# LingmaFuture/PRCV2025REID

Hardware: AMD Instinct MI355X
Metric: multimodal instances/sec (PxK, 5-modality) at 1/2/4/8 GPU; eval queries/sec (higher is better)
Workload: dtype bf16; 1 GPU; P=16,K=4 per GPU, vis/nir/sk/cp 224x224 + text (T<=77), CLIP ViT-B/16 + text tower random-init, MER-LoRA r=8, masks all-on, 400 ids, SDM+CE, fwd+bwd+grad sanitise/clip+AdamW (reference default trainable set); P=16, K=4, global_batch=64, lora_rank=8, accum_steps=1, parallelism=dp1

## Files before the change

include/reid_hip.h:

```cpp
#ifndef REID_HIP_H
#define REID_HIP_H

#include <stdint.h>

#ifdef __cplusplus
extern "C" {
#endif

typedef enum {
    REID_OK = 0,
    REID_ERR_ARG = -1,
    REID_ERR_LAUNCH = -2,
    REID_ERR_DEVICE = -3
} reid_status;

typedef enum { REID_BF16 = 0, REID_F32 = 1, REID_F16 = 2 } reid_dtype;

typedef enum {
    REID_ACT_NONE = 0,
    REID_ACT_GELU_ERF = 1,
    REID_ACT_QUICK_GELU = 2,
    REID_ACT_RELU = 3,
    REID_ACT_DGELU_ERF = 4,
    REID_ACT_DQUICK_GELU = 5,
// ... 69 lines not shown

int reid_attn_fwd(const void* qkv, int32_t ld, const uint8_t* key_mask, void* out, int32_t ldo, float* lse,
                  int32_t n_seq, int32_t S, int32_t heads, int32_t causal, int32_t q_tiles, void* stream);
int reid_attn_bwd(const void* qkv, int32_t ld, const uint8_t* key_mask, const void* out, const void* dout,
                  int32_t ldo, const float* lse, void* dqkv, int32_t lddqkv, float* delta_ws,
                  int32_t n_seq, int32_t S, int32_t heads, int32_t causal, int32_t q_tiles, void* stream);

int reid_cast_f32_bf16(const float* src, void* dst, int64_t n, void* stream);
int reid_cast_bf16_f32(const void* src, float* dst, int64_t n, void* stream);
int reid_pack_bf16_table(const float* src, void* dst_bf16, const int64_t* table, int32_t n_entries, void* stream);
int reid_lora_bwd_fused(const void* dY, int32_t lddy, const void* T, int32_t ldt, const void* BT, int32_t ldbt, void* U, int32_t ldu,
                        float* dB, int32_t lddb, const int32_t* img_mod, int32_t rows_per_img, int32_t mask_r, int32_t M, int32_t N,
                        int32_t Rp, float scale, float* u_partial, int32_t u_mode, void* stream);
int reid_lora_da_fused(const void* X, int32_t ldx, const void* U, int32_t ldu, float* dA, int32_t ldda, const int32_t* img_mod,
                       int32_t rows_per_img, int32_t mask_r, int32_t M, int32_t K, int32_t Rp, int32_t n_groups, void* stream);

int reid_merge_lora_table(const int64_t* table, int32_t n_entries, int32_t max_tiles, const float* arena, void* weff,
                          int32_t Rp, int32_t r, int32_t nmod, float scaling, void* stream);
int reid_gather_rows_f32(const float* src, int32_t lds, const int32_t* index, float* dst, int32_t ldd,
                         int32_t rows, int32_t cols, void* stream);
int reid_embed_tokens(const float* tok, const float* pos, const int64_t* ids, float* out, int32_t B, int32_t T, int32_t D,
                      int32_t vocab, void* stream);
int reid_scatter_add_rows_f32(const float* src, int32_t lds, const int32_t* index, float* out, int32_t ldo,
                              int32_t rows, int32_t cols, int32_t out_rows, void* stream);

int reid_bnneck_stats(const float* x, int32_t ldx, int32_t rows, int32_t D, float* sum, float* sqsum, void* stream);
int reid_bnneck_fwd(const float* x, int32_t ldx, const float* gamma, const float* beta, float* running_mean,
                    float* running_var, const float* sum, const float* sqsum, float count, int32_t training,
                    float* y, void* y_bf16, int32_t ldy, float* mean, float* invstd, float* rnorm,
                    int32_t rows, int32_t D, float eps, float momentum, float scale, void* stream);
// ... 224 lines not shown
```

prcv2025reid_amd/_lib.py:

```python
import ctypes as C
import os

import torch

_HERE = os.path.dirname(os.path.abspath(__file__))
LIB_PATHS = {'bf16': os.path.join(_HERE, 'csrc', 'libreid_hip.so'), 'f16': os.path.join(_HERE, 'csrc', 'libreid_hip_f16.so')}
if os.environ.get('REID_LIB_BF16'):
    LIB_PATHS['bf16'] = os.environ['REID_LIB_BF16']
LIB_PATH = LIB_PATHS['bf16']
T16_DTYPES = {'bf16': torch.bfloat16, 'f16': torch.float16}
_flavor = os.environ.get('REID_T16', 'bf16')


def set_flavor(name: str):
    global _flavor
    if name not in LIB_PATHS:
        raise ValueError(f'unknown 16-bit flavor {name!r}')
    _flavor = name


def flavor() -> str:
    return _flavor


# ... 45 lines not shown
    'reid_mer_gemm': (_I, [_GEMM, _P]),
    'reid_mer_gemm_plan': (_I, [_GEMM, _I, _I, _PLAN]),
    'reid_gemm_tn': (_I, [_P, _P, _P, _I, _I, _I, _I, _I, _I, _F, _F, _P]),
    'reid_layernorm_fwd': (_I, [_P, _I, _P, _P, _P, _P, _P, _I, _P, _P, _I, _I, _F, _P]),
    'reid_add_layernorm_fwd': (_I, [_P, _I, _P, _I, _I, _P, _I, _P, _I, _P, _P, _P, _I, _P, _P, _I, _I, _F, _P]),
    'reid_layernorm_bwd': (_I, [_P, _I, _I, _P, _I, _P, _P, _P, _P, _P, _P, _I, _P, _I, _P, _P, _I, _I, _P, _I, _P, _P]),
    'reid_patch_im2col': (_I, [_P, _P, _I, _I, _I, _I, _I, _P]),
    'reid_cls_rows': (_I, [_P, _P, _P, _I, _I, _I, _I, _P]),
    'reid_attn_fwd': (_I, [_P, _I, _P, _P, _I, _P, _I, _I, _I, _I, _I, _P]),
    'reid_attn_bwd': (_I, [_P, _I, _P, _P, _P, _I, _P, _P, _I, _P, _I, _I, _I, _I, _I, _P]),
    'reid_cast_f32_bf16': (_I, [_P, _P, _I64, _P]),
    'reid_cast_bf16_f32': (_I, [_P, _P, _I64, _P]),
    'reid_pack_bf16_table': (_I, [_P, _P, _P, _I, _P]),
    'reid_lora_bwd_fused': (_I, [_P, _I, _P, _I, _P, _I, _P, _I, _P, _I, _P, _I, _I, _I, _I, _I, _F, _P, _I, _P]),
    'reid_lora_da_fused': (_I, [_P, _I, _P, _I, _P, _I, _P, _I, _I, _I, _I, _I, _I, _P]),
    'reid_merge_lora_table': (_I, [_P, _I, _I, _P, _P, _I, _I, _I, _F, _P]),
    'reid_gather_rows_f32': (_I, [_P, _I, _P, _P, _I, _I, _I, _P]),
    'reid_embed_tokens': (_I, [_P, _P, _P, _P, _I, _I, _I, _I, _P]),
    'reid_scatter_add_rows_f32': (_I, [_P, _I, _P, _P, _I, _I, _I, _I, _P]),
    'reid_bnneck_stats': (_I, [_P, _I, _I, _I, _P, _P, _P]),
    'reid_bnneck_fwd': (_I, [_P, _I, _P, _P, _P, _P, _P, _P, _F, _I, _P, _P, _I, _P, _P, _P, _I, _I, _F, _F, _F, _P]),
    'reid_bnneck_bwd_p1': (_I, [_P, _I, _P, _I, _P, _P, _P, _P, _P, _P, _P, _P, _I, _I, _F, _P]),
    'reid_bnneck_bwd_p2': (_I, [_P, _P, _I, _P, _P, _P, _P, _P, _F, _I, _P, _I, _I, _I, _P]),
    'reid_ce_ls_fwd': (_I, [_P, _I, _P, _P, _I, _I, _F, _P, _P, _P]),
    'reid_ce_ls_bwd': (_I, [_P, _I, _P, _P, _I, _I, _F, _P, _P, _I, _P]),
    'reid_sdm_fwd': (_I, [_P, _I, _P, _I, _P, _P, _P, _P, _I, _I, _I, _I, _F, _P, _P, _P]),
    'reid_sdm_bwd': (_I, [_P, _I, _P, _I, _P, _P, _P, _P, _I, _I, _I, _I, _F, _P, _P, _P, _I, _P, _I, _P]),
    'reid_sdm_ws_floats': (_I64, [_I, _I, _I, _I]),
    'reid_triplet_hard_fwd': (_I, [_P, _I, _P, _P, _I, _I, _F, _P, _P, _P, _P, _P, _P, _P]),
    'reid_triplet_hard_bwd': (_I, [_P, _I, _I, _I, _F, _P, _P, _P, _P, _P, _P, _P, _I, _P]),
# ... 147 lines not shown
```

prcv2025reid_amd/csrc/lora.hip:

```cpp
#include "lds_tile.h"
#include <type_traits>

namespace {
using namespace ldstile;

constexpr int MT = 64;

__global__ __launch_bounds__(256) void merge_lora_kernel(const int64_t* __restrict__ table, const float* __restrict__ arena,
                                                         bf16_t* __restrict__ weff, int Rp, int r, int nmod, float s) {
    REID_T16_ENTER();
    const int64_t* e = table + (size_t)blockIdx.y * 8;
    const int N = (int)e[5], K = (int)e[6], G = (int)e[7];
    const int tiles_k = K / MT;
    if ((int)blockIdx.x >= (N / MT) * tiles_k) return;
    const float* __restrict__ W = (const float*)e[0];
    const float* __restrict__ A = arena + e[1];
    const float* __restrict__ B = arena + e[2];
    bf16_t* dst = weff + e[3];
    bf16_t* dstT = e[4] >= 0 ? weff + e[4] : nullptr;
    const int n0 = ((int)blockIdx.x / tiles_k) * MT, k0 = ((int)blockIdx.x % tiles_k) * MT;
    const int g = n0 / (N / G);
    const int R = nmod * r;
    __shared__ __attribute__((aligned(16))) float sW[MT][MT + 4];
    __shared__ __attribute__((aligned(16))) float sA[MT][MT + 4];
// ... 274 lines not shown
    return buf + 1 == NBUF ? 0 : buf + 1;
}

__global__ __launch_bounds__(256) void u_finish_kernel(const float* __restrict__ Up, bf16_t* __restrict__ U, int ldu, const int32_t* __restrict__ img_mod,
                                                       int rows_per_img, int mask_r, float scale, int M, int Rp) {
    REID_T16_ENTER();
    const int i = blockIdx.x * 256 + threadIdx.x;
    const int h = Rp >> 1;
    const int m = i / h, c = (i - m * h) * 2;
    if (m >= M) return;
    const int mu = img_mod[m / rows_per_img];
    const float a = Up[(size_t)m * Rp + c], b = Up[(size_t)m * Rp + c + 1];
    *(uint32_t*)(U + (size_t)m * ldu + c) = pack_bf16x2(c / mask_r == mu ? a * scale : 0.f, (c + 1) / mask_r == mu ? b * scale : 0.f);
}

template <int RP>
__device__ __forceinline__ void lora_bwd_image_run(const Params& p, char* smem, const int rbeg, const int rend, const int mu) {
    constexpr int BUF_BYTES = BwdGeo<RP>::BUF_BYTES;
    int tid = threadIdx.x;
    asm volatile("" : "+v"(tid));
    const int lane = tid & 63;
    const int w = __builtin_amdgcn_readfirstlane(tid >> 6);
    const int l16 = lane & 15, fq = lane >> 4;
    const int w0 = (mu * p.mask_r) & ~15;
    const int c_lo = mu * p.mask_r - w0, c_hi = c_lo + p.mask_r;
    const int steps = (rend - rbeg + R - 1) / R;
    const uint32_t smem_a = lds_addr(smem);
    auto issue = [&](int t, int buf) {
        const uint32_t base = smem_a + buf * BUF_BYTES;
        const int r0 = rbeg + t * R;
        dma_tile(p.dY, p.lddy, r0, rend, w, lane, base);
        if constexpr (RP == 32) {
            if (w < 2) {
                const int g = w * 64 + lane;
                const int row = g >> 2, c = g & 3;
                int gr = r0 + row; gr = gr < rend ? gr : rend - 1;
                dma16(p.T + (size_t)gr * p.ldt + c * 8, base + IMG_BYTES + w * 1024);
            }
        } else {
            if (w == 0) {
                const int row = lane >> 1, c = lane & 1;
                int gr = r0 + row; gr = gr < rend ? gr : rend - 1;
                dma16(p.T + (size_t)gr * p.ldt + w0 + c * 8, base + IMG_BYTES);
            }
        }
    };
    ring_prologue(steps, issue);
    bf16x8 bfr[24];
    if (w < 2) {
#pragma unroll
        for (int ks = 0; ks < 24; ++ks) bfr[ks] = *(const bf16x8*)(p.BT + (size_t)(w0 + l16) * p.ldbt + ks * 32 + 8 * fq);
#pragma unroll
        for (int ks = 0; ks < 24; ++ks) asm volatile("" ::"v"(bfr[ks]));
    }
    f32x4 acc[8];
#pragma unroll
    for (int i = 0; i < 8; ++i) acc[i] = f32x4{0.f, 0.f, 0.f, 0.f};
    typedef unsigned u32x4_t __attribute__((ext_vector_type(4)));
    u32x4_t pend_val = u32x4_t{0u, 0u, 0u, 0u};
    u32x4_t pend_val2 = u32x4_t{0u, 0u, 0u, 0u};
    void* pend_ptr = nullptr;
    int pend_n = 0;
    if constexpr (RP == 64) {
        if (w < 2 && p.u_mode == 0) {
            char* ub = smem + NBUF * BUF_BYTES + w * (16 * RP * 2);
            *(u32x4_t*)(ub + lane * 16) = u32x4_t{0u, 0u, 0u, 0u};
            *(u32x4_t*)(ub + 1024 + lane * 16) = u32x4_t{0u, 0u, 0u, 0u};
        }
    }
    auto flush_pending = [&]() {
        if (p.u_mode == 0) {
            if constexpr (RP == 32) {
                if (pend_n) asm volatile("global_store_dwordx4 %0, %1, off" ::"v"(pend_ptr), "v"(pend_val) : "memory");
            } else {
                if (pend_n & 1) asm volatile("global_store_dwordx4 %0, %1, off" ::"v"(pend_ptr), "v"(pend_val) : "memory");
                if (pend_n & 2) {
                    void* pp2 = (void*)((bf16_t*)pend_ptr + (size_t)8 * p.ldu);
                    asm volatile("global_store_dwordx4 %0, %1, off" ::"v"(pp2), "v"(pend_val2) : "memory");
                }
            }
        } else {
#pragma unroll
            for (int e = 0; e < 4; ++e) {
                if (e >= pend_n) continue;
                float* pp = (float*)pend_ptr + (size_t)e * RP;
                const unsigned vv = pend_val[e];
                if (p.u_mode == 2) asm volatile("global_store_dword %0, %1, off" ::"v"(pp), "v"(vv) : "memory");
                else asm volatile("global_atomic_add_f32 %0, %1, off" ::"v"(pp), "v"(vv) : "memory");
            }
        }
        pend_n = 0;
    };
    int buf = 0;
    for (int t = 0; t < steps; ++t) {
        ring_wait(t, steps, w < (RP == 32 ? 2 : 1));
        const char* xs = smem + buf * BUF_BYTES;
        const char* ts = xs + IMG_BYTES;
        const int r0 = rbeg + t * R;
        if (w < 2) {
            flush_pending();
            f32x4 u4[4];
#pragma unroll
            for (int a = 0; a < 4; ++a) u4[a] = f32x4{0.f, 0.f, 0.f, 0.f};
            const int row = 16 * w + l16;
            const char* xrow = xs + row * ROW_BYTES;
#pragma unroll
            for (int k0 = 0; k0 < 24; k0 += 4) {
                bf16x8 af[4];
#pragma unroll
                for (int a = 0; a < 4; ++a) af[a] = *(const bf16x8*)(xrow + (swz512(row, 4 * (k0 + a) + fq) << 4));
#pragma unroll
                for (int a = 0; a < 4; ++a) u4[a] = mfma16(af[a], bfr[k0 + a], u4[a]);
            }
            const f32x4 ua = (u4[0] + u4[1]) + (u4[2] + u4[3]);
// ... 28 lines not shown
        } else {
            bf16x8 tf = RP == 32 ? tr_frag(ts, RP * 2, 0, w0, lane) : tr_frag(ts, 32, 0, 0, lane);
            const int nvalid = rend - r0;
            if (nvalid < R) {
#pragma unroll
                for (int j = 0; j < 8; ++j) {
                    if (16 * (j >> 2) + 4 * fq + (j & 3) >= nvalid) tf[j] = 0;
                }
            }
            const int cbase = (w - 2) * 128;
#pragma unroll
            for (int i = 0; i < 8; ++i) acc[i] = mfma16(tr_frag_swz(xs, cbase + i * 16, lane), tf, acc[i]);
        }
        buf = ring_refill(t, steps, buf, issue);
    }
    if (w < 2) flush_pending();
    __syncthreads();
    int ftid = threadIdx.x;
    asm volatile("" : "+v"(ftid));
    float* fl = (float*)smem;
    if (w >= 2) {
        const int cbase = (w - 2) * 128, fl16 = ftid & 15, ffq = (ftid & 63) >> 4;
#pragma unroll
        for (int i = 0; i < 8; ++i)
#pragma unroll
            for (int e = 0; e < 4; ++e) fl[(cbase + i * 16 + 4 * ffq + e) * 16 + fl16] = acc[i][e];
    }
    __syncthreads();
    {
        const int rr = p.mask_r, total = N * rr;
        for (int idx = ftid; idx < total; idx += 512) {
            const int col = idx / rr, j = idx - col * rr;
            atomicAdd(p.dB + (size_t)col * p.lddb + mu * rr + j, fl[col * 16 + c_lo + j]);
        }
    }
}

template <int RP>
__global__ __launch_bounds__(512, 2) void lora_bwd_image_kernel(const Params p) {
    REID_T16_ENTER();
    static_assert(RP == 32 || RP == 64, "adapter columns");
    extern __shared__ __attribute__((aligned(16))) char smem[];
    for_each_run(p, [=](int rbeg, int rend, int mu, bool more) { lora_bwd_image_run<RP>(p, smem, rbeg, rend, mu); if (more) __syncthreads(); });
}

struct DaParams {
    const bf16_t* X; const bf16_t* U; float* dA;
    const int32_t* img_mod;
    int ldx, ldu, ldda, rows_per_img, mask_r, M, Rp, span, n_img;
};
template <int G>
__device__ __forceinline__ void lora_da_image_run(const DaParams& p, char* smem, const int rbeg, const int rend, const int mu, const bool more) {
    constexpr int UB = 4096;
    constexpr int BUF = IMG_BYTES + UB;
    const int tid = threadIdx.x, lane = tid & 63;
    const int w = __builtin_amdgcn_readfirstlane(tid >> 6);
    const int l16 = lane & 15, fq = lane >> 4;
    const int cblk = blockIdx.y;
    const int w0 = (mu * p.mask_r) & ~15;
    const int c_lo = mu * p.mask_r - w0, c_hi = c_lo + p.mask_r;
    const int steps = (rend - rbeg + R - 1) / R;
    const bf16_t* Xb = p.X + (size_t)cblk * N;
    const uint32_t smem_a = lds_addr(smem);
    auto issue = [&](int t, int buf) {
        const uint32_t base = smem_a + buf * BUF;
        const int r0 = rbeg + t * R;
        dma_tile(Xb, p.ldx, r0, rend, w, lane, base);
        if (w < G) {
            const int row = lane >> 1, c = lane & 1;
            int gr = r0 + row; gr = gr < rend ? gr : rend - 1;
            dma16(p.U + (size_t)gr * p.ldu + w * p.Rp + w0 + c * 8, base + IMG_BYTES + w * 1024);
        }
    };
    ring_prologue(steps, issue);
    f32x4 acc[G][6];
#pragma unroll
    for (int g = 0; g < G; ++g)
#pragma unroll
        for (int i = 0; i < 6; ++i) acc[g][i] = f32x4{0.f, 0.f, 0.f, 0.f};
    int buf = 0;
    for (int t = 0; t < steps; ++t) {
        ring_wait(t, steps, w < G);
        const char* xs = smem + buf * BUF;
        const char* us = xs + IMG_BYTES;
        const int nvalid = rend - (rbeg + t * R);
        bf16x8 uf[G];
#pragma unroll
        for (int g = 0; g < G; ++g) {
            uf[g] = tr_frag(us + g * 1024, 32, 0, 0, lane);
            if (nvalid < R) {
#pragma unroll
                for (int j = 0; j < 8; ++j)
                    if (16 * (j >> 2) + 4 * fq + (j & 3) >= nvalid) uf[g][j] = 0;
            }
        }
#pragma unroll
        for (int i = 0; i < 6; ++i) {
            const bf16x8 xf = tr_frag_swz(xs, w * 96 + i * 16, lane);
#pragma unroll
            for (int g = 0; g < G; ++g) acc[g][i] = mfma16(uf[g], xf, acc[g][i]);
        }
        buf = ring_refill(t, steps, buf, issue);
    }
    if (more) __syncthreads();
#pragma unroll
    for (int e = 0; e < 4; ++e) {
        const int c = 4 * fq + e;
        if (c < c_lo || c >= c_hi) continue;
#pragma unroll
        for (int g = 0; g < G; ++g)
#pragma unroll
            for (int i = 0; i < 6; ++i)
                atomicAdd(p.dA + (size_t)(g * p.Rp + w0 + c) * p.ldda + (size_t)cblk * N + w * 96 + i * 16 + l16, acc[g][i][e]);
    }
}

template <int G>
__global__ __launch_bounds__(512, 2) void lora_da_image_kernel(const DaParams p) {
    REID_T16_ENTER();
    extern __shared__ __attribute__((aligned(16))) char smem[];
    for_each_run(p, [=](int rbeg, int rend, int mu, bool more) { lora_da_image_run<G>(p, smem, rbeg, rend, mu, more); });
}
}

}

static int lora_span(int n_img) {
    const int k = reid_knob(KNOB_LORA_SPAN);
    if (k == 1 || k == 2 || k == 4 || k == 8) return k;
    return n_img >= reid_num_cus() ? 4 : 1;
}

static bool lora_image_shape(int rows_per_img, int mask_r) { return rows_per_img >= image::R && mask_r <= 16 && 16 % mask_r == 0; }

extern "C" int reid_lora_bwd_fused(const void* dY, int32_t lddy, const void* T, int32_t ldt, const void* BT, int32_t ldbt, void* U,
                                   int32_t ldu, float* dB, int32_t lddb, const int32_t* img_mod, int32_t rows_per_img, int32_t mask_r,
                                   int32_t M, int32_t N, int32_t Rp, float scale, float* u_partial, int32_t u_mode, void* stream) {
    REID_CHECK_ARG(u_mode >= 0 && u_mode <= 3 && (u_mode == 0 || u_partial), "reid_lora_bwd_fused: u_mode=%d needs u_partial", u_mode);
    REID_CHECK_ARG(dY && T && BT && U && dB && img_mod, "reid_lora_bwd_fused: null pointer");
    REID_CHECK_ARG(N == fused::N && (Rp == 32 || Rp == 64), "reid_lora_bwd_fused: N=%d Rp=%d (this kernel is built for N = 768, Rp = 32 or 64)", N, Rp);
    REID_CHECK_ARG(M > 0 && rows_per_img > 0 && mask_r > 0 && mask_r <= Rp, "reid_lora_bwd_fused: M=%d rows_per_img=%d mask_r=%d", M, rows_per_img, mask_r);
    REID_CHECK_ARG(lddy % 8 == 0 && ldt % 8 == 0 && ldbt % 8 == 0 && ldu % 2 == 0 && lddy >= N && ldt >= Rp && ldbt >= N && ldu >= Rp && lddb >= Rp,
                   "reid_lora_bwd_fused: leading dimensions");
    REID_CHECK_ARG(((uintptr_t)dY | (uintptr_t)T | (uintptr_t)BT) % 16 == 0 && (uintptr_t)U % 4 == 0, "reid_lora_bwd_fused: operand alignment");
    fused::Params p{(const bf16_t*)dY, (const bf16_t*)T, (const bf16_t*)BT, (bf16_t*)U, dB, img_mod, lddy, ldt, ldbt, ldu, lddb, rows_per_img,
                    mask_r, M, 0, scale, u_partial, u_mode, 1, 0};
    const bool use_image = reid_knob(KNOB_LORA_IMPL) != 1 && lora_image_shape(rows_per_img, mask_r);
    REID_CHECK_ARG(Rp == 32 || use_image, "reid_lora_bwd_fused: Rp=64 runs one image per workgroup only: rows_per_img=%d must be >= 32, mask_r=%d a "
                   "divisor of 16, and REID_LORA_IMPL not 1 (the slab kernel is built for Rp = 32)", rows_per_img, mask_r);
    if (use_image) {
        const int n_img = (M + rows_per_img - 1) / rows_per_img;
        p.n_img = n_img;
        p.span = lora_span(n_img);
        const int grid = (n_img + p.span - 1) / p.span;
        if (Rp == 32) {
            REID_MAX_LDS((image::lora_bwd_image_kernel<32>), image::BwdGeo<32>::LDS_BYTES);
            hipLaunchKernelGGL(image::lora_bwd_image_kernel<32>, dim3(grid), dim3(512), image::BwdGeo<32>::LDS_BYTES, (hipStream_t)stream, p);
        } else {
            REID_MAX_LDS((image::lora_bwd_image_kernel<64>), image::BwdGeo<64>::LDS_BYTES);
            hipLaunchKernelGGL(image::lora_bwd_image_kernel<64>, dim3(grid), dim3(512), image::BwdGeo<64>::LDS_BYTES, (hipStream_t)stream, p);
        }
        REID_CHECK_LAUNCH("reid_lora_bwd_fused(image)");
        if (u_mode == 1) {
            hipLaunchKernelGGL(image::u_finish_kernel, dim3((M * (Rp / 2) + 255) / 256), dim3(256), 0, (hipStream_t)stream, (const float*)u_partial, (bf16_t*)U,
                               ldu, img_mod, rows_per_img, mask_r, scale, M, Rp);
            REID_CHECK_LAUNCH("reid_lora_bwd_fused(finish)");
        }
        return REID_OK;
    }
    int slabs = 64;
    p.slab_rows = ((M + slabs - 1) / slabs + fused::R - 1) / fused::R * fused::R;
    slabs = (M + p.slab_rows - 1) / p.slab_rows;
    REID_MAX_LDS(fused::lora_bwd_fused_kernel, fused::LDS_BYTES);
    hipLaunchKernelGGL(fused::lora_bwd_fused_kernel, dim3(slabs), dim3(fused::NW * 64), fused::LDS_BYTES, (hipStream_t)stream, p);
    REID_CHECK_LAUNCH("reid_lora_bwd_fused");
    return REID_OK;
}

extern "C" int reid_lora_da_fused(const void* X, int32_t ldx, const void* U, int32_t ldu, float* dA, int32_t ldda, const int32_t* img_mod,
                                  int32_t rows_per_img, int32_t mask_r, int32_t M, int32_t K, int32_t Rp, int32_t n_groups, void* stream) {
    REID_CHECK_ARG(X && U && dA && img_mod, "reid_lora_da_fused: null pointer");
    REID_CHECK_ARG(M > 0 && K > 0 && K % 768 == 0 && (Rp == 32 || Rp == 64) && (n_groups == 1 || n_groups == 3), "reid_lora_da_fused: M=%d K=%d Rp=%d groups=%d (K a multiple of 768, Rp = 32 or 64, 1 or 3 groups)", M, K, Rp, n_groups);
    REID_CHECK_ARG(mask_r > 0 && lora_image_shape(rows_per_img, mask_r), "reid_lora_da_fused: rows_per_img=%d (>= 32) mask_r=%d (a divisor of 16)", rows_per_img, mask_r);
    REID_CHECK_ARG(ldx % 8 == 0 && ldu % 8 == 0 && ldx >= K && ldu >= n_groups * Rp && ldda >= K, "reid_lora_da_fused: leading dimensions");
    REID_CHECK_ARG(((uintptr_t)X | (uintptr_t)U) % 16 == 0, "reid_lora_da_fused: operand alignment");
    const int n_img = (M + rows_per_img - 1) / rows_per_img;
    const int span = lora_span(n_img);
    image::DaParams p{(const bf16_t*)X, (const bf16_t*)U, dA, img_mod, ldx, ldu, ldda, rows_per_img, mask_r, M, Rp, span, n_img};
    const dim3 grid((n_img + span - 1) / span, K / 768);
    constexpr int LDS = image::NBUF * (image::IMG_BYTES + 4096);
    if (n_groups == 1) {
        REID_MAX_LDS((image::lora_da_image_kernel<1>), LDS);
        hipLaunchKernelGGL(image::lora_da_image_kernel<1>, grid, dim3(512), LDS, (hipStream_t)stream, p);
    } else {
        REID_MAX_LDS((image::lora_da_image_kernel<3>), LDS);
        hipLaunchKernelGGL(image::lora_da_image_kernel<3>, grid, dim3(512), LDS, (hipStream_t)stream, p);
    }
    REID_CHECK_LAUNCH("reid_lora_da_fused");
    return REID_OK;
}

extern "C" int reid_merge_lora_table(const int64_t* table, int32_t n_entries, int32_t max_tiles, const float* arena, void* weff,
                                     int32_t Rp, int32_t r, int32_t nmod, float scaling, void* stream) {
    REID_CHECK_ARG(table && arena && weff, "reid_merge_lora_table: null pointer");
    REID_CHECK_ARG(n_entries > 0 && n_entries <= 65535 && max_tiles > 0, "reid_merge_lora_table: n_entries=%d max_tiles=%d", n_entries, max_tiles);
    REID_CHECK_ARG(r > 0 && nmod > 0 && r <= MT && nmod * r <= Rp, "reid_merge_lora_table: r = %d must be <= %d and nmod*r = %d <= Rp = %d", r, MT, nmod * r, Rp);
    hipLaunchKernelGGL(merge_lora_kernel, dim3(max_tiles, n_entries), dim3(256), 0, (hipStream_t)stream, table, arena, (bf16_t*)weff, Rp, r, nmod,
                       scaling);
    REID_CHECK_LAUNCH("reid_merge_lora_table");
    return REID_OK;
}
```

prcv2025reid_amd/engine.py:

```python
from types import SimpleNamespace
from typing import Dict, List, Optional, Tuple

import math
import os

import torch

from . import _lib, ops

LIN = ('qkv', 'out', 'fc1', 'fc2')
REF_LIN = {'attn.q_proj': ('qkv', 0), 'attn.k_proj': ('qkv', 1), 'attn.v_proj': ('qkv', 2), 'attn.out_proj': ('out', 0),
           'mlp.fc1': ('fc1', 0), 'mlp.fc2': ('fc2', 0)}


def round_up(a, b):
    return (a + b - 1) // b * b


def grad_scale(amax):
    return torch.exp2(torch.floor(torch.log2(512.0 / amax))).clamp(2.0 ** -20, 2.0 ** 40)


class DenseGrads:

# ... 341 lines not shown
                if yb is None:
                    yb = buf['yb'] = torch.empty(M, d, dtype=torch.float16, device=dev)
                ops.gemm(oin, we(l, 'out'), yb, bias=P[lp + 'attn.out_proj.shared_linear.bias'], row_groups=rg)
                ops.add_layernorm_fwd(xin, yb, xm, P[lp + 'ln2.weight'], P[lp + 'ln2.bias'], h2, mean2, rstd2, row_scale=sa, rows_per_img=rpi)
            else:
                ops.gemm(oin, we(l, 'out'), xm, bias=P[lp + 'attn.out_proj.shared_linear.bias'], R=xin, row_scale=sa, rows_per_img=rpi,
                         row_groups=rg)
                ops.layernorm_fwd(xm, P[lp + 'ln2.weight'], P[lp + 'ln2.bias'], y_bf16=h2, mean=mean2, rstd=rstd2)
            u = new('u', (Mr, ff), b16) if save else None
            g = new('g', (Mr, ff), b16)
            ops.gemm(h2, we(l, 'fc1'), g, bias=P[lp + 'mlp.fc1.shared_linear.bias'], act='gelu_dsave' if save else 'gelu', C2=u,
                     row_groups=rg)
            T = To = T1 = T2 = None
            if save:
                T = torch.empty(M, 3 * Rp, **b16); To = torch.empty(Mr, Rp, **b16)
                T1 = torch.empty(Mr, Rp, **b16); T2 = torch.empty(Mr, Rp, **b16)
                lora_down([(h, pk(l, 'qkv', 'A'), T, full.mask), (oin, pk(l, 'out', 'A'), To, rows.mask),
                           (h2, pk(l, 'fc1', 'A'), T1, rows.mask), (g, pk(l, 'fc2', 'A'), T2, rows.mask)])
            xn = torch.empty(Mr, d, **f32) if save else new('xn' + str(l & 1) + ('c' if last else ''), (Mr, d), f32)
            if not last:
                np_ = f'{ce}vision_layers.{l + 1}.'
                ops.gemm(g, we(l, 'fc2'), yb, bias=P[lp + 'mlp.fc2.shared_linear.bias'], row_groups=rg)
                nxt = (new('h' + str((l + 1) & 1), (M, d), b16), new('m1' + str((l + 1) & 1), (M,), f32), new('r1' + str((l + 1) & 1), (M,), f32))
                ops.add_layernorm_fwd(xm, yb, xn, P[np_ + 'ln1.weight'], P[np_ + 'ln1.bias'], nxt[0], nxt[1], nxt[2], row_scale=sm_,
                                      rows_per_img=rpi)
            else:
                ops.gemm(g, we(l, 'fc2'), xn, bias=P[lp + 'mlp.fc2.shared_linear.bias'], R=xm, row_scale=sm_, rows_per_img=rpi,
                         row_groups=rg)
            if save:
                saved.append(dict(x=x, h=h, mean1=mean1, rstd1=rstd1, T=T, qkv=qkv, o=o, lse=lse, To=To, xm=xm, h2=h2,
                                  mean2=mean2, rstd2=rstd2, T1=T1, u=u, g=g, T2=T2, sa=sa, sm=sm_, cls=last, o_rows=oin))
            x = xn
        cls_h = torch.empty(n_img, d, **b16); mf = torch.empty(n_img, **f32); rf = torch.empty(n_img, **f32)
# ... 47 lines not shown
        U2 = torch.empty(M, Rp, **b16); U1 = torch.empty(M, Rp, **b16); Uo = torch.empty(M, Rp, **b16)
        Uq = torch.empty(M, 3 * Rp, **b16)
        du2 = [torch.empty(M, ff, **b16) for _ in range(2)]
        dqkv2 = [torch.empty(M, 3 * d, **b16) for _ in range(2)]
        dxmb2 = [torch.empty(M, d, **b16) for _ in range(2)]
        dxb2 = [dxb, torch.empty(M, d, **b16)]
        dh = torch.empty(M, d, **b16); do = torch.empty(M, d, **b16)
        delta = torch.empty(n_img, heads, S, **f32)
        dxm = torch.empty(M, d, **gx)
        weT = lambda l, nm: lay.weff(self._weff, l, nm, transposed=True)
        main = torch.cuda.current_stream(dev)
        side = self._side_stream() if self.overlap_tn else None
        side_done = {}
        L = a['vision_layers']
        u_part = torch.empty(M, Rp, **f32)
        rows_full, rows_cls = st['rows']
        full = SimpleNamespace(**vars(rows_full), gy=dx, gyb=dxb2, U2=U2, U1=U1, Uo=Uo, du=du2, dh=dh, do=do, dxm=dxm, dxmb=dxmb2)
        cls = SimpleNamespace(**vars(rows_cls), gy=dx_c, gyb=[dxb_c] * 2,
                              U2=torch.empty(n_img, Rp, **b16), U1=torch.empty(n_img, Rp, **b16), Uo=torch.empty(n_img, Rp, **b16),
                              du=[torch.empty(n_img, ff, **b16)] * 2, dh=torch.empty(n_img, d, **b16), do=torch.empty(n_img, d, **b16),
                              dxm=torch.empty(n_img, d, **gx), dxmb=[torch.empty(n_img, d, **b16)] * 2)

        def adapter_grads(l, nm, dY, X, T, U, rows):
            if side is not None:
                wait_for(side, main)
            with torch.cuda.stream(side):
                BT, dB = pk(l, nm, 'BT'), lay.view_B(grad, l, nm)
                G = lay.ent[(l, nm)]['G']
                n = dY.shape[1] // G
                for g in range(G):
                    dYg, Tg, BTg, Ug, dBg = dY[:, g * n:(g + 1) * n], T[:, g * Rp:(g + 1) * Rp], BT[:, g * n:(g + 1) * n], \
                        U[:, g * Rp:(g + 1) * Rp], dB[g * n:(g + 1) * n]
                    if ops.lora_bwd_fused_ok(n, Rp, rows.rpi, r):
                        ops.lora_bwd_fused(dYg, Tg, BTg, Ug, dBg, rows.img_mod, rows.rpi, r, self.scaling,
                                           u_partial=u_part[:dY.shape[0]] if n > 768 else None)
                    else:
                        ops.gemm(dYg, BTg, Ug, **rows.mask)
                        ops.gemm_tn(dYg, Tg, dBg, beta=1.0)
                if ops.lora_da_fused_ok(X.shape[1], Rp, rows.rpi, r, G):
                    ops.lora_da_fused(X, U, lay.view_A(grad, l, nm), rows.img_mod, rows.rpi, r, n_groups=G)
                else:
                    ops.gemm_tn(U, X, lay.view_A(grad, l, nm), beta=1.0)

# ... 270 lines not shown
```

prcv2025reid_amd/ops.py:

```python
import ctypes as C
from typing import Optional

import torch

from . import _lib as L
from ._lib import BF16, F32, GemmArgs, GemmPlan, check, lib, ptr, stream_ptr

ACT = {'none': L.ACT_NONE, 'gelu': L.ACT_GELU, 'quick_gelu': L.ACT_QUICK_GELU, 'relu': L.ACT_RELU,
       'dgelu': L.ACT_DGELU, 'dquick_gelu': L.ACT_DQUICK_GELU, 'drelu': L.ACT_DRELU,
       'mul_aux': L.ACT_MUL_AUX, 'gelu_dsave': L.ACT_GELU_DSAVE}


_gemm_profile = None
def gemm_profile_begin():
    global _gemm_profile
    _gemm_profile = []


def gemm_profile_end():
    global _gemm_profile
    p, _gemm_profile = _gemm_profile, None
    return p


# ... 143 lines not shown


def cast_f32_bf16(src, dst):
    check(lib().reid_cast_f32_bf16(ptr(src), ptr(dst), src.numel(), stream_ptr()))
    return dst


def cast_bf16_f32(src, dst):
    check(lib().reid_cast_bf16_f32(ptr(src), ptr(dst), src.numel(), stream_ptr()))
    return dst


def lora_bwd_fused(dY, T, BT, U, dB, img_mod, rows_per_img, mask_r, scale, u_partial=None):
    N = dY.shape[1]
    nb = N // 768
    if nb > 1 and u_partial is None:
        raise ValueError('lora_bwd_fused: a cotangent wider than 768 columns needs u_partial')
    for q in range(nb):
        mode = 0 if nb == 1 else ((1 if q > 0 else 0) | (2 if q + 1 < nb else 0))
        dYq, BTq, dBq = dY[:, q * 768:(q + 1) * 768], BT[:, q * 768:(q + 1) * 768], dB[q * 768:(q + 1) * 768]
        check(lib().reid_lora_bwd_fused(ptr(dYq), dYq.stride(0), ptr(T), T.stride(0), ptr(BTq), BTq.stride(0), ptr(U), U.stride(0),
                                        ptr(dBq), dBq.stride(0), ptr(img_mod), rows_per_img, mask_r, dY.shape[0], 768, T.shape[1],
                                        scale, ptr(u_partial), mode, stream_ptr()))


def lora_da_fused(X, U, dA, img_mod, rows_per_img, mask_r, n_groups=1):
    check(lib().reid_lora_da_fused(ptr(X), X.stride(0), ptr(U), U.stride(0), ptr(dA), dA.stride(0), ptr(img_mod), rows_per_img, mask_r,
                                   X.shape[0], X.shape[1], U.shape[1] // n_groups, n_groups, stream_ptr()))


def lora_da_fused_ok(K, Rp, rows_per_img, mask_r, n_groups):
    return K % 768 == 0 and Rp in (32, 64) and rows_per_img >= 32 and mask_r <= 16 and 16 % mask_r == 0 and n_groups in (1, 3)


def lora_bwd_fused_ok(N, Rp, rows_per_img=None, mask_r=None):
    if N % 768 != 0 or N // 768 not in (1, 2, 3, 4):
        return False
    if Rp == 32:
        return True
    return Rp == 64 and rows_per_img is not None and mask_r is not None and rows_per_img >= 32 and 0 < mask_r <= 16 and 16 % mask_r == 0


def merge_lora_table(table, n_entries, max_tiles, arena, weff, Rp, r, nmod, scaling):
# ... 749 lines not shown
```

Before: 2176 instances/s.

## Recompute fc2 LoRA down-projection inside dA backward kernel instead of saving it

The forward pass no longer saves the fc2 LoRA down-projection T2 when the shape allows it. In backward, U is computed first, then the dA kernel re-reads X from LDS and also forms T = A·X into fp32 partials, which a small finish kernel reduces and masks. A dB-only pass of the bwd kernel follows. This removes a forward down-projection and its activation storage, at the cost of splitting the backward into three kernels and adding MFMA work inside the dA kernel.

Result: no change. 2197 instances/s, median of 6 (+1.0%).

```diff
diff --git a/include/reid_hip.h b/include/reid_hip.h
--- a/include/reid_hip.h
+++ b/include/reid_hip.h
@@ -107,6 +107,9 @@
                         int32_t Rp, float scale, float* u_partial, int32_t u_mode, void* stream);
 int reid_lora_da_fused(const void* X, int32_t ldx, const void* U, int32_t ldu, float* dA, int32_t ldda, const int32_t* img_mod,
                        int32_t rows_per_img, int32_t mask_r, int32_t M, int32_t K, int32_t Rp, int32_t n_groups, void* stream);
+int reid_lora_da_t_fused(const void* X, int32_t ldx, const void* U, int32_t ldu, float* dA, int32_t ldda, const void* A, int32_t lda,
+                         void* T, int32_t ldt, float* t_partial, float scale, const int32_t* img_mod, int32_t rows_per_img,
+                         int32_t mask_r, int32_t M, int32_t K, int32_t Rp, void* stream);
 
 int reid_merge_lora_table(const int64_t* table, int32_t n_entries, int32_t max_tiles, const float* arena, void* weff,
                           int32_t Rp, int32_t r, int32_t nmod, float scaling, void* stream);
diff --git a/prcv2025reid_amd/_lib.py b/prcv2025reid_amd/_lib.py
--- a/prcv2025reid_amd/_lib.py
+++ b/prcv2025reid_amd/_lib.py
@@ -83,6 +83,7 @@
     'reid_pack_bf16_table': (_I, [_P, _P, _P, _I, _P]),
     'reid_lora_bwd_fused': (_I, [_P, _I, _P, _I, _P, _I, _P, _I, _P, _I, _P, _I, _I, _I, _I, _I, _F, _P, _I, _P]),
     'reid_lora_da_fused': (_I, [_P, _I, _P, _I, _P, _I, _P, _I, _I, _I, _I, _I, _I, _P]),
+    'reid_lora_da_t_fused': (_I, [_P, _I, _P, _I, _P, _I, _P, _I, _P, _I, _P, _F, _P, _I, _I, _I, _I, _I, _P]),
     'reid_merge_lora_table': (_I, [_P, _I, _I, _P, _P, _I, _I, _I, _F, _P]),
     'reid_gather_rows_f32': (_I, [_P, _I, _P, _P, _I, _I, _I, _P]),
     'reid_embed_tokens': (_I, [_P, _P, _P, _P, _I, _I, _I, _I, _P]),
diff --git a/prcv2025reid_amd/csrc/lora.hip b/prcv2025reid_amd/csrc/lora.hip
--- a/prcv2025reid_amd/csrc/lora.hip
+++ b/prcv2025reid_amd/csrc/lora.hip
@@ -312,7 +312,8 @@
     *(uint32_t*)(U + (size_t)m * ldu + c) = pack_bf16x2(c / mask_r == mu ? a * scale : 0.f, (c + 1) / mask_r == mu ? b * scale : 0.f);
 }
 
-template <int RP>
+enum { BOTH = 0, U_ONLY = 1, DB_ONLY = 2 };
+template <int RP, int MODE>
 __device__ __forceinline__ void lora_bwd_image_run(const Params& p, char* smem, const int rbeg, const int rend, const int mu) {
     constexpr int BUF_BYTES = BwdGeo<RP>::BUF_BYTES;
     int tid = threadIdx.x;
@@ -328,7 +329,8 @@
         const uint32_t base = smem_a + buf * BUF_BYTES;
         const int r0 = rbeg + t * R;
         dma_tile(p.dY, p.lddy, r0, rend, w, lane, base);
-        if constexpr (RP == 32) {
+        if constexpr (MODE == U_ONLY) {
+        } else if constexpr (RP == 32) {
             if (w < 2) {
                 const int g = w * 64 + lane;
                 const int row = g >> 2, c = g & 3;
@@ -345,7 +347,7 @@
     };
     ring_prologue(steps, issue);
     bf16x8 bfr[24];
-    if (w < 2) {
+    if (MODE != DB_ONLY && w < 2) {
 #pragma unroll
         for (int ks = 0; ks < 24; ++ks) bfr[ks] = *(const bf16x8*)(p.BT + (size_t)(w0 + l16) * p.ldbt + ks * 32 + 8 * fq);
 #pragma unroll
@@ -360,7 +362,7 @@
     void* pend_ptr = nullptr;
     int pend_n = 0;
     if constexpr (RP == 64) {
-        if (w < 2 && p.u_mode == 0) {
+        if (MODE != DB_ONLY && w < 2 && p.u_mode == 0) {
             char* ub = smem + NBUF * BUF_BYTES + w * (16 * RP * 2);
             *(u32x4_t*)(ub + lane * 16) = u32x4_t{0u, 0u, 0u, 0u};
             *(u32x4_t*)(ub + 1024 + lane * 16) = u32x4_t{0u, 0u, 0u, 0u};
@@ -391,11 +393,13 @@
     };
     int buf = 0;
     for (int t = 0; t < steps; ++t) {
-        ring_wait(t, steps, w < (RP == 32 ? 2 : 1));
+        ring_wait(t, steps, MODE != U_ONLY && w < (RP == 32 ? 2 : 1));
         const char* xs = smem + buf * BUF_BYTES;
         const char* ts = xs + IMG_BYTES;
         const int r0 = rbeg + t * R;
-        if (w < 2) {
+        if (MODE == DB_ONLY && w < 2) {
+        } else if (MODE == U_ONLY && w >= 2) {
+        } else if (w < 2) {
             flush_pending();
             f32x4 u4[4];
 #pragma unroll
@@ -454,7 +458,8 @@
         }
         buf = ring_refill(t, steps, buf, issue);
     }
-    if (w < 2) flush_pending();
+    if (MODE != DB_ONLY && w < 2) flush_pending();
+    if constexpr (MODE == U_ONLY) return;
     __syncthreads();
     int ftid = threadIdx.x;
     asm volatile("" : "+v"(ftid));
@@ -476,21 +481,23 @@
     }
 }
 
-template <int RP>
+template <int RP, int MODE>
 __global__ __launch_bounds__(512, 2) void lora_bwd_image_kernel(const Params p) {
     REID_T16_ENTER();
     static_assert(RP == 32 || RP == 64, "adapter columns");
     extern __shared__ __attribute__((aligned(16))) char smem[];
-    for_each_run(p, [=](int rbeg, int rend, int mu, bool more) { lora_bwd_image_run<RP>(p, smem, rbeg, rend, mu); if (more) __syncthreads(); });
+    for_each_run(p, [=](int rbeg, int rend, int mu, bool more) { lora_bwd_image_run<RP, MODE>(p, smem, rbeg, rend, mu); if (more) __syncthreads(); });
 }
 
 struct DaParams {
     const bf16_t* X; const bf16_t* U; float* dA;
     const int32_t* img_mod;
     int ldx, ldu, ldda, rows_per_img, mask_r, M, Rp, span, n_img;
+    const bf16_t* A; float* Tp; int lda;
 };
-template <int G>
+template <int G, bool WT>
 __device__ __forceinline__ void lora_da_image_run(const DaParams& p, char* smem, const int rbeg, const int rend, const int mu, const bool more) {
+    static_assert(!WT || G == 1, "T is formed beside one adapter group");
     constexpr int UB = 4096;
     constexpr int BUF = IMG_BYTES + UB;
     const int tid = threadIdx.x, lane = tid & 63;
@@ -513,6 +520,23 @@
         }
     };
     ring_prologue(steps, issue);
+    typedef unsigned u32x4_t __attribute__((ext_vector_type(4)));
+    bf16x8 afr[WT ? 24 : 1];
+    u32x4_t pend_val = u32x4_t{0u, 0u, 0u, 0u};
+    void* pend_ptr = nullptr;
+    int pend_n = 0;
+    if constexpr (WT) {
+        if (w < 2) {
+#pragma unroll
+            for (int ks = 0; ks < 24; ++ks) afr[ks] = *(const bf16x8*)(p.A + (size_t)(w0 + l16) * p.lda + (size_t)cblk * N + ks * 32 + 8 * fq);
+#pragma unroll
+            for (int ks = 0; ks < 24; ++ks) asm volatile("" ::"v"(afr[ks]));
+        }
+    }
+    auto flush_pending = [&]() {
+        if (pend_n) asm volatile("global_store_dwordx4 %0, %1, off" ::"v"(pend_ptr), "v"(pend_val) : "memory");
+        pend_n = 0;
+    };
     f32x4 acc[G][6];
 #pragma unroll
     for (int g = 0; g < G; ++g)
@@ -524,6 +548,29 @@
         const char* xs = smem + buf * BUF;
         const char* us = xs + IMG_BYTES;
         const int nvalid = rend - (rbeg + t * R);
+        if constexpr (WT) {
+            if (w < 2) {
+                flush_pending();
+                f32x4 t4[4];
+#pragma unroll
+                for (int a = 0; a < 4; ++a) t4[a] = f32x4{0.f, 0.f, 0.f, 0.f};
+                const int row = 16 * w + l16;
+                const char* xrow = xs + row * ROW_BYTES;
+#pragma unroll
+                for (int k0 = 0; k0 < 24; k0 += 4) {
+                    bf16x8 xf[4];
+#pragma unroll
+                    for (int a = 0; a < 4; ++a) xf[a] = *(const bf16x8*)(xrow + (swz512(row, 4 * (k0 + a) + fq) << 4));
+#pragma unroll
+                    for (int a = 0; a < 4; ++a) t4[a] = mfma16(afr[k0 + a], xf[a], t4[a]);
+                }
+                const f32x4 ta = (t4[0] + t4[1]) + (t4[2] + t4[3]);
+                const int m = rbeg + t * R + row;
+                pend_val = u32x4_t{__float_as_uint(ta[0]), __float_as_uint(ta[1]), __float_as_uint(ta[2]), __float_as_uint(ta[3])};
+                pend_ptr = (void*)(p.Tp + ((size_t)cblk * p.M + m) * 16 + 4 * fq);
+                pend_n = m < rend ? 1 : 0;
+            }
+        }
         bf16x8 uf[G];
 #pragma unroll
         for (int g = 0; g < G; ++g) {
@@ -542,6 +589,9 @@
         }
         buf = ring_refill(t, steps, buf, issue);
     }
+    if constexpr (WT) {
+        if (w < 2) flush_pending();
+    }
     if (more) __syncthreads();
 #pragma unroll
     for (int e = 0; e < 4; ++e) {
@@ -555,11 +605,30 @@
     }
 }
 
-template <int G>
+template <int G, bool WT>
 __global__ __launch_bounds__(512, 2) void lora_da_image_kernel(const DaParams p) {
     REID_T16_ENTER();
     extern __shared__ __attribute__((aligned(16))) char smem[];
-    for_each_run(p, [=](int rbeg, int rend, int mu, bool more) { lora_da_image_run<G>(p, smem, rbeg, rend, mu, more); });
+    for_each_run(p, [=](int rbeg, int rend, int mu, bool more) { lora_da_image_run<G, WT>(p, smem, rbeg, rend, mu, more); });
+}
+
+__global__ __launch_bounds__(256) void t_finish_kernel(const float* __restrict__ Tp, bf16_t* __restrict__ T, int ldt, const int32_t* __restrict__ img_mod,
+                                                       int rows_per_img, int mask_r, float scale, int M, int Rp, int nblk) {
+    REID_T16_ENTER();
+    const int i = blockIdx.x * 256 + threadIdx.x;
+    const int h = Rp >> 1;
+    const int m = i / h, c = (i - m * h) * 2;
+    if (m >= M) return;
+    const int mu = img_mod[m / rows_per_img];
+    const int w0 = (mu * mask_r) & ~15;
+    float a = 0.f, b = 0.f;
+    if (c >= w0 && c < w0 + 16) {
+        for (int q = 0; q < nblk; ++q) {
+            const float* t = Tp + ((size_t)q * M + m) * 16 + (c - w0);
+            a += t[0]; b += t[1];
+        }
+    }
+    *(uint32_t*)(T + (size_t)m * ldt + c) = pack_bf16x2(c / mask_r == mu ? a * scale : 0.f, (c + 1) / mask_r == mu ? b * scale : 0.f);
 }
 }
 
@@ -576,16 +645,19 @@
 extern "C" int reid_lora_bwd_fused(const void* dY, int32_t lddy, const void* T, int32_t ldt, const void* BT, int32_t ldbt, void* U,
                                    int32_t ldu, float* dB, int32_t lddb, const int32_t* img_mod, int32_t rows_per_img, int32_t mask_r,
                                    int32_t M, int32_t N, int32_t Rp, float scale, float* u_partial, int32_t u_mode, void* stream) {
-    REID_CHECK_ARG(u_mode >= 0 && u_mode <= 3 && (u_mode == 0 || u_partial), "reid_lora_bwd_fused: u_mode=%d needs u_partial", u_mode);
-    REID_CHECK_ARG(dY && T && BT && U && dB && img_mod, "reid_lora_bwd_fused: null pointer");
+    const bool u_only = u_mode == 4, db_only = u_mode == 8;
+    REID_CHECK_ARG(u_only || db_only || (u_mode >= 0 && u_mode <= 3 && (u_mode == 0 || u_partial)), "reid_lora_bwd_fused: u_mode=%d (0-3, 4 or 8; 1-3 need u_partial)", u_mode);
+    REID_CHECK_ARG(dY && img_mod && (u_only || (T && dB)) && (db_only || (BT && U)), "reid_lora_bwd_fused: null pointer");
     REID_CHECK_ARG(N == fused::N && (Rp == 32 || Rp == 64), "reid_lora_bwd_fused: N=%d Rp=%d (this kernel is built for N = 768, Rp = 32 or 64)", N, Rp);
     REID_CHECK_ARG(M > 0 && rows_per_img > 0 && mask_r > 0 && mask_r <= Rp, "reid_lora_bwd_fused: M=%d rows_per_img=%d mask_r=%d", M, rows_per_img, mask_r);
-    REID_CHECK_ARG(lddy % 8 == 0 && ldt % 8 == 0 && ldbt % 8 == 0 && ldu % 2 == 0 && lddy >= N && ldt >= Rp && ldbt >= N && ldu >= Rp && lddb >= Rp,
+    REID_CHECK_ARG(lddy % 8 == 0 && lddy >= N && (u_only || (ldt % 8 == 0 && ldt >= Rp && lddb >= Rp)) && (db_only || (ldbt % 8 == 0 && ldu % 2 == 0 && ldbt >= N && ldu >= Rp)),
                    "reid_lora_bwd_fused: leading dimensions");
     REID_CHECK_ARG(((uintptr_t)dY | (uintptr_t)T | (uintptr_t)BT) % 16 == 0 && (uintptr_t)U % 4 == 0, "reid_lora_bwd_fused: operand alignment");
     fused::Params p{(const bf16_t*)dY, (const bf16_t*)T, (const bf16_t*)BT, (bf16_t*)U, dB, img_mod, lddy, ldt, ldbt, ldu, lddb, rows_per_img,
-                    mask_r, M, 0, scale, u_partial, u_mode, 1, 0};
+                    mask_r, M, 0, scale, u_partial, (u_only || db_only) ? 0 : u_mode, 1, 0};
     const bool use_image = reid_knob(KNOB_LORA_IMPL) != 1 && lora_image_shape(rows_per_img, mask_r);
+    REID_CHECK_ARG(use_image || !(u_only || db_only), "reid_lora_bwd_fused: u_mode=%d runs one image per workgroup only (rows_per_img=%d >= 32, mask_r=%d a divisor "
+                   "of 16, REID_LORA_IMPL not 1)", u_mode, rows_per_img, mask_r);
     REID_CHECK_ARG(Rp == 32 || use_image, "reid_lora_bwd_fused: Rp=64 runs one image per workgroup only: rows_per_img=%d must be >= 32, mask_r=%d a "
                    "divisor of 16, and REID_LORA_IMPL not 1 (the slab kernel is built for Rp = 32)", rows_per_img, mask_r);
     if (use_image) {
@@ -593,13 +665,21 @@
         p.n_img = n_img;
         p.span = lora_span(n_img);
         const int grid = (n_img + p.span - 1) / p.span;
+#define REID_LAUNCH_BWD_IMAGE(RP_, MODE_)                                                                                          \
+    do {                                                                                                                          \
+        REID_MAX_LDS((image::lora_bwd_image_kernel<RP_, image::MODE_>), image::BwdGeo<RP_>::LDS_BYTES);                               \
+        hipLaunchKernelGGL((image::lora_bwd_image_kernel<RP_, image::MODE_>), dim3(grid), dim3(512), image::BwdGeo<RP_>::LDS_BYTES, (hipStream_t)stream, p); \
+    } while (0)
         if (Rp == 32) {
-            REID_MAX_LDS((image::lora_bwd_image_kernel<32>), image::BwdGeo<32>::LDS_BYTES);
-            hipLaunchKernelGGL(image::lora_bwd_image_kernel<32>, dim3(grid), dim3(512), image::BwdGeo<32>::LDS_BYTES, (hipStream_t)stream, p);
+            if (u_only) REID_LAUNCH_BWD_IMAGE(32, U_ONLY);
+            else if (db_only) REID_LAUNCH_BWD_IMAGE(32, DB_ONLY);
+            else REID_LAUNCH_BWD_IMAGE(32, BOTH);
         } else {
-            REID_MAX_LDS((image::lora_bwd_image_kernel<64>), image::BwdGeo<64>::LDS_BYTES);
-            hipLaunchKernelGGL(image::lora_bwd_image_kernel<64>, dim3(grid), dim3(512), image::BwdGeo<64>::LDS_BYTES, (hipStream_t)stream, p);
-        }
+            if (u_only) REID_LAUNCH_BWD_IMAGE(64, U_ONLY);
+            else if (db_only) REID_LAUNCH_BWD_IMAGE(64, DB_ONLY);
+            else REID_LAUNCH_BWD_IMAGE(64, BOTH);
+        }
+#undef REID_LAUNCH_BWD_IMAGE
         REID_CHECK_LAUNCH("reid_lora_bwd_fused(image)");
         if (u_mode == 1) {
             hipLaunchKernelGGL(image::u_finish_kernel, dim3((M * (Rp / 2) + 255) / 256), dim3(256), 0, (hipStream_t)stream, (const float*)u_partial, (bf16_t*)U,
@@ -626,17 +706,40 @@
     REID_CHECK_ARG(((uintptr_t)X | (uintptr_t)U) % 16 == 0, "reid_lora_da_fused: operand alignment");
     const int n_img = (M + rows_per_img - 1) / rows_per_img;
     const int span = lora_span(n_img);
-    image::DaParams p{(const bf16_t*)X, (const bf16_t*)U, dA, img_mod, ldx, ldu, ldda, rows_per_img, mask_r, M, Rp, span, n_img};
+    image::DaParams p{(const bf16_t*)X, (const bf16_t*)U, dA, img_mod, ldx, ldu, ldda, rows_per_img, mask_r, M, Rp, span, n_img, nullptr, nullptr, 0};
     const dim3 grid((n_img + span - 1) / span, K / 768);
     constexpr int LDS = image::NBUF * (image::IMG_BYTES + 4096);
     if (n_groups == 1) {
-        REID_MAX_LDS((image::lora_da_image_kernel<1>), LDS);
-        hipLaunchKernelGGL(image::lora_da_image_kernel<1>, grid, dim3(512), LDS, (hipStream_t)stream, p);
+        REID_MAX_LDS((image::lora_da_image_kernel<1, false>), LDS);
+        hipLaunchKernelGGL((image::lora_da_image_kernel<1, false>), grid, dim3(512), LDS, (hipStream_t)stream, p);
     } else {
-        REID_MAX_LDS((image::lora_da_image_kernel<3>), LDS);
-        hipLaunchKernelGGL(image::lora_da_image_kernel<3>, grid, dim3(512), LDS, (hipStream_t)stream, p);
+        REID_MAX_LDS((image::lora_da_image_kernel<3, false>), LDS);
+        hipLaunchKernelGGL((image::lora_da_image_kernel<3, false>), grid, dim3(512), LDS, (hipStream_t)stream, p);
     }
     REID_CHECK_LAUNCH("reid_lora_da_fused");
+    return REID_OK;
+}
+
+extern "C" int reid_lora_da_t_fused(const void* X, int32_t ldx, const void* U, int32_t ldu, float* dA, int32_t ldda, const void* A, int32_t lda,
+                                    void* T, int32_t ldt, float* t_partial, float scale, const int32_t* img_mod, int32_t rows_per_img,
+                                    int32_t mask_r, int32_t M, int32_t K, int32_t Rp, void* stream) {
+    REID_CHECK_ARG(X && U && dA && A && T && t_partial && img_mod, "reid_lora_da_t_fused: null pointer");
+    REID_CHECK_ARG(M > 0 && K > 0 && K % 768 == 0 && (Rp == 32 || Rp == 64), "reid_lora_da_t_fused: M=%d K=%d Rp=%d (K a multiple of 768, Rp = 32 or 64)", M, K, Rp);
+    REID_CHECK_ARG(mask_r > 0 && lora_image_shape(rows_per_img, mask_r), "reid_lora_da_t_fused: rows_per_img=%d (>= 32) mask_r=%d (a divisor of 16)", rows_per_img, mask_r);
+    REID_CHECK_ARG(ldx % 8 == 0 && ldu % 8 == 0 && lda % 8 == 0 && ldt % 2 == 0 && ldx >= K && ldu >= Rp && ldda >= K && lda >= K && ldt >= Rp,
+                   "reid_lora_da_t_fused: leading dimensions");
+    REID_CHECK_ARG(((uintptr_t)X | (uintptr_t)U | (uintptr_t)A | (uintptr_t)t_partial) % 16 == 0 && (uintptr_t)T % 4 == 0, "reid_lora_da_t_fused: operand alignment");
+    const int n_img = (M + rows_per_img - 1) / rows_per_img;
+    const int span = lora_span(n_img);
+    image::DaParams p{(const bf16_t*)X, (const bf16_t*)U, dA, img_mod, ldx, ldu, ldda, rows_per_img, mask_r, M, Rp, span, n_img, (const bf16_t*)A, t_partial, lda};
+    const dim3 grid((n_img + span - 1) / span, K / 768);
+    constexpr int LDS = image::NBUF * (image::IMG_BYTES + 4096);
+    REID_MAX_LDS((image::lora_da_image_kernel<1, true>), LDS);
+    hipLaunchKernelGGL((image::lora_da_image_kernel<1, true>), grid, dim3(512), LDS, (hipStream_t)stream, p);
+    REID_CHECK_LAUNCH("reid_lora_da_t_fused");
+    hipLaunchKernelGGL(image::t_finish_kernel, dim3((M * (Rp / 2) + 255) / 256), dim3(256), 0, (hipStream_t)stream, (const float*)t_partial, (bf16_t*)T, ldt,
+                       img_mod, rows_per_img, mask_r, scale, M, Rp, K / 768);
+    REID_CHECK_LAUNCH("reid_lora_da_t_fused(finish)");
     return REID_OK;
 }
 
diff --git a/prcv2025reid_amd/engine.py b/prcv2025reid_amd/engine.py
--- a/prcv2025reid_amd/engine.py
+++ b/prcv2025reid_amd/engine.py
@@ -379,9 +379,12 @@
             T = To = T1 = T2 = None
             if save:
                 T = torch.empty(M, 3 * Rp, **b16); To = torch.empty(Mr, Rp, **b16)
-                T1 = torch.empty(Mr, Rp, **b16); T2 = torch.empty(Mr, Rp, **b16)
-                lora_down([(h, pk(l, 'qkv', 'A'), T, full.mask), (oin, pk(l, 'out', 'A'), To, rows.mask),
-                           (h2, pk(l, 'fc1', 'A'), T1, rows.mask), (g, pk(l, 'fc2', 'A'), T2, rows.mask)])
+                T1 = torch.empty(Mr, Rp, **b16)
+                calls = [(h, pk(l, 'qkv', 'A'), T, full.mask), (oin, pk(l, 'out', 'A'), To, rows.mask), (h2, pk(l, 'fc1', 'A'), T1, rows.mask)]
+                if not ops.lora_da_t_ok(d, ff, Rp, rpi, self.lay.r):
+                    T2 = torch.empty(Mr, Rp, **b16)
+                    calls.append((g, pk(l, 'fc2', 'A'), T2, rows.mask))
+                lora_down(calls)
             xn = torch.empty(Mr, d, **f32) if save else new('xn' + str(l & 1) + ('c' if last else ''), (Mr, d), f32)
             if not last:
                 np_ = f'{ce}vision_layers.{l + 1}.'
@@ -459,6 +462,7 @@
         side_done = {}
         L = a['vision_layers']
         u_part = torch.empty(M, Rp, **f32)
+        T2b = torch.empty(M, Rp, **b16); t_part = torch.empty((ff // 768) * M * 16, **f32)
         rows_full, rows_cls = st['rows']
         full = SimpleNamespace(**vars(rows_full), gy=dx, gyb=dxb2, U2=U2, U1=U1, Uo=Uo, du=du2, dh=dh, do=do, dxm=dxm, dxmb=dxmb2)
         cls = SimpleNamespace(**vars(rows_cls), gy=dx_c, gyb=[dxb_c] * 2,
@@ -472,6 +476,12 @@
             with torch.cuda.stream(side):
                 BT, dB = pk(l, nm, 'BT'), lay.view_B(grad, l, nm)
                 G = lay.ent[(l, nm)]['G']
+                if T is None:
+                    ops.lora_u(dY, BT, U, rows.img_mod, rows.rpi, r, self.scaling)
+                    ops.lora_da_fused(X, U, lay.view_A(grad, l, nm), rows.img_mod, rows.rpi, r, A=pk(l, nm, 'A'), T=T2b, t_partial=t_part,
+                                      scale=self.scaling)
+                    ops.lora_bwd_fused(dY, T2b, None, None, dB, rows.img_mod, rows.rpi, r, self.scaling)
+                    return
                 n = dY.shape[1] // G
                 for g in range(G):
                     dYg, Tg, BTg, Ug, dBg = dY[:, g * n:(g + 1) * n], T[:, g * Rp:(g + 1) * Rp], BT[:, g * n:(g + 1) * n], \
diff --git a/prcv2025reid_amd/ops.py b/prcv2025reid_amd/ops.py
--- a/prcv2025reid_amd/ops.py
+++ b/prcv2025reid_amd/ops.py
@@ -181,6 +181,12 @@
 def lora_bwd_fused(dY, T, BT, U, dB, img_mod, rows_per_img, mask_r, scale, u_partial=None):
     N = dY.shape[1]
     nb = N // 768
+    if BT is None:
+        if U is not None or nb != 1:
+            raise ValueError('lora_bwd_fused: dB alone takes a 768-column cotangent and neither BT nor U')
+        check(lib().reid_lora_bwd_fused(ptr(dY), dY.stride(0), ptr(T), T.stride(0), None, 0, None, 0, ptr(dB), dB.stride(0), ptr(img_mod),
+                                        rows_per_img, mask_r, dY.shape[0], 768, T.shape[1], scale, None, 8, stream_ptr()))
+        return
     if nb > 1 and u_partial is None:
         raise ValueError('lora_bwd_fused: a cotangent wider than 768 columns needs u_partial')
     for q in range(nb):
@@ -191,9 +197,25 @@
                                         scale, ptr(u_partial), mode, stream_ptr()))
 
 
-def lora_da_fused(X, U, dA, img_mod, rows_per_img, mask_r, n_groups=1):
-    check(lib().reid_lora_da_fused(ptr(X), X.stride(0), ptr(U), U.stride(0), ptr(dA), dA.stride(0), ptr(img_mod), rows_per_img, mask_r,
-                                   X.shape[0], X.shape[1], U.shape[1] // n_groups, n_groups, stream_ptr()))
+def lora_u(dY, BT, U, img_mod, rows_per_img, mask_r, scale):
+    check(lib().reid_lora_bwd_fused(ptr(dY), dY.stride(0), None, 0, ptr(BT), BT.stride(0), ptr(U), U.stride(0), None, 0, ptr(img_mod),
+                                    rows_per_img, mask_r, dY.shape[0], dY.shape[1], U.shape[1], scale, None, 4, stream_ptr()))
+
+
+def lora_da_fused(X, U, dA, img_mod, rows_per_img, mask_r, n_groups=1, A=None, T=None, t_partial=None, scale=1.0):
+    if T is None:
+        check(lib().reid_lora_da_fused(ptr(X), X.stride(0), ptr(U), U.stride(0), ptr(dA), dA.stride(0), ptr(img_mod), rows_per_img, mask_r,
+                                       X.shape[0], X.shape[1], U.shape[1] // n_groups, n_groups, stream_ptr()))
+        return
+    M, K = X.shape
+    if n_groups != 1 or A is None or t_partial is None or t_partial.dtype != torch.float32 or t_partial.numel() < (K // 768) * M * 16:
+        raise ValueError('lora_da_fused: T needs one group, A, and t_partial of (K / 768) * M * 16 fp32 elements')
+    check(lib().reid_lora_da_t_fused(ptr(X), X.stride(0), ptr(U), U.stride(0), ptr(dA), dA.stride(0), ptr(A), A.stride(0), ptr(T), T.stride(0),
+                                     ptr(t_partial), scale, ptr(img_mod), rows_per_img, mask_r, M, K, U.shape[1], stream_ptr()))
+
+
+def lora_da_t_ok(N, K, Rp, rows_per_img, mask_r):
+    return N == 768 and K > N and lora_da_fused_ok(K, Rp, rows_per_img, mask_r, 1) and lora_bwd_fused_ok(N, Rp, rows_per_img, mask_r)
 
 
 def lora_da_fused_ok(K, Rp, rows_per_img, mask_r, n_groups):
```
